# tensorlayer/HyperPose

Hardware: AMD Instinct MI355X
Metric: end-to-end FPS (preproc+DNN+PAF parse) @ 368x432 (higher is better)
Workload: dtype f32; 1 GPU; configs[1]: Lightweight-OpenPose (MobilenetDilated) + PAF parser, batch 8 @ 368x432 per GPU; frames from pinned host memory (one H2D per batch), parser on the network's own maps, humans to the host; key=configs[1]/f32, global_batch=8, parallelism=frame-sharded x1, no steady-state collective, pipes_per_gpu=4, parser_input=the network's own heat-maps

## Files before the change

hyperpose_amd/csrc/conv32_head.hip:

```cpp
#include "conv_fp32.hpp"

#include "conv_device.hpp"

#include <cstdlib>

namespace hp {

namespace {

typedef float f32x4 __attribute__((ext_vector_type(4)));

constexpr int HK1 = 128;
constexpr int HXP = (HK1 + 4) * 4;
constexpr int HX_BYTES = 32 * HXP;

__device__ __forceinline__ long tvh_off(const tview32& t, int b, int y, int x)
{
    return ((long)b * t.img + (long)y * t.wp + x) * t.cs + t.coff;
}

}

template <int TM2>
__device__ __forceinline__ void conv32_head_body(const conv32_params& q, const head32_hidden& h, unsigned char* const xs, float* const red_, const int blk)
{
    float (*const red)[TM2][4][64][4] = reinterpret_cast<float (*)[TM2][4][64][4]>(red_);

    const int tid = threadIdx.x, lane = tid & 63, wave = tid >> 6;
    const int n0 = blk * 32;
    const int OHW = q.OH * q.OW;

    {
        const int px = tid >> 3, q0 = tid & 7;
        const int n = min(n0 + px, q.npix - 1);
        const int b = n / OHW, rem = n - b * OHW;
        const int oy = rem / q.OW, ox = rem - oy * q.OW;
        const float* const src = q.in.p + tvh_off(q.in, b, oy, ox);
        f32x4 v[4];
#pragma unroll
        for (int i = 0; i < 4; ++i)
            v[i] = *reinterpret_cast<const f32x4*>(src + (q0 + 8 * i) * 4);
#pragma unroll
        for (int i = 0; i < 4; ++i)
            *reinterpret_cast<f32x4*>(xs + px * HXP + (q0 + 8 * i) * 16) = v[i];
    }
    lds_barrier();
    const int n = lane & 31, fk = lane >> 5;
    f32x4 xb[HK1 / 8];
#pragma unroll
    for (int k = 0; k < HK1 / 8; ++k)
        xb[k] = *reinterpret_cast<const f32x4*>(xs + n * HXP + (k * 8 + fk * 4) * 4);

    floatx16 acc2[TM2];
#pragma unroll
    for (int m = 0; m < TM2; ++m)
#pragma unroll
        for (int r = 0; r < 16; ++r)
            acc2[m][r] = 0.f;

    const int MT1 = h.HID / 32, nt = MT1 / 4;
    const float* const w1 = h.w1_frag + lane * 4;
    const float* const w2 = h.w2_frag + lane * 4;
    constexpr int KS = HK1 / 8, RING = 4, AHEAD = 3;
    const int nsteps = nt * KS;
    f32x4 fa[RING];
    auto aload = [&](int slot, int st) {
        const int sc = min(st, nsteps - 1), ht = wave + 4 * (sc / KS), k = sc % KS;
        fa[slot] = *reinterpret_cast<const f32x4*>(w1 + (long)(k * MT1 + ht) * 256);
    };
#pragma unroll
    for (int a = 0; a < AHEAD; ++a)
        aload(a, a);
#pragma unroll 1
    for (int it = 0; it < nt; ++it) {
        const int ht = wave + 4 * it;
        floatx16 acc1;
#pragma unroll
        for (int r = 0; r < 16; ++r)
            acc1[r] = 0.f;
        f32x4 a2[TM2][4];
#pragma unroll
        for (int m = 0; m < TM2; ++m)
#pragma unroll
            for (int qd = 0; qd < 4; ++qd)
                a2[m][qd] = *reinterpret_cast<const f32x4*>(w2 + (long)(((ht * TM2 + m) * 4 + qd) * 256));
        f32x4 bs[4];
#pragma unroll
        for (int qd = 0; qd < 4; ++qd)
            bs[qd] = *reinterpret_cast<const f32x4*>(h.bias1 + ht * 32 + 8 * qd + 4 * fk);
#pragma unroll
        for (int k = 0; k < KS; ++k) {
            aload((k + AHEAD) % RING, it * KS + k + AHEAD);
            const f32x4 a = fa[k % RING];
#pragma unroll
            for (int e = 0; e < 4; ++e)
                acc1 = __builtin_amdgcn_mfma_f32_32x32x2f32(a[e], xb[k][e], acc1, 0, 0, 0);
        }
#pragma unroll
        for (int r = 0; r < 16; ++r) {
            const float x = acc1[r] + bs[r >> 2][r & 3];
            acc1[r] = x > 0.f ? fminf(x, h.hi1) : x * h.slope1;
        }
#pragma unroll
        for (int m = 0; m < TM2; ++m)
#pragma unroll
            for (int r = 0; r < 16; ++r)
                acc2[m] = __builtin_amdgcn_mfma_f32_32x32x2f32(a2[m][r >> 2][r & 3], acc1[r], acc2[m], 0, 0, 0);
    }

#pragma unroll
    for (int m = 0; m < TM2; ++m)
#pragma unroll
        for (int qd = 0; qd < 4; ++qd)
            *reinterpret_cast<f32x4*>(&red[wave][m][qd][lane][0]) = f32x4{ acc2[m][4 * qd], acc2[m][4 * qd + 1], acc2[m][4 * qd + 2], acc2[m][4 * qd + 3] };
    lds_barrier();
    if (wave >= TM2)
        return;
    const int np = n0 + n;
    const bool pix_ok = np < q.npix;
    const int nc = min(np, q.npix - 1);
    const int b = nc / OHW, rem = nc - b * OHW;
    const int oy = rem / q.OW, ox = rem - oy * q.OW;
    const long ooff = q.out.p ? tvh_off(q.out, b, oy, ox) : 0;
    const bool out_vec = q.out.p && ((q.out.coff | q.out.cs) & 3) == 0;
#pragma unroll
    for (int qd = 0; qd < 4; ++qd) {
        f32x4 sum = *reinterpret_cast<const f32x4*>(&red[0][wave][qd][lane][0]);
#pragma unroll
        for (int w = 1; w < 4; ++w)
            sum += *reinterpret_cast<const f32x4*>(&red[w][wave][qd][lane][0]);
        const int m = wave * 32 + 8 * qd + 4 * fk;
        if (pix_ok && m < q.Cout) {
            const bool full = m + 3 < q.Cout;
            const f32x4 b2 = *reinterpret_cast<const f32x4*>(q.bias + m);
            f32x4 sl = { q.act_slope, q.act_slope, q.act_slope, q.act_slope };
            if (q.alpha)
                sl = *reinterpret_cast<const f32x4*>(q.alpha + m);
            float v[4];
#pragma unroll
            for (int e = 0; e < 4; ++e) {
                const float x = sum[e] + b2[e];
                v[e] = x > 0.f ? fminf(x, q.act_hi) : x * sl[e];
            }
            if (q.out.p) {
                if (full && out_vec)
                    *reinterpret_cast<f32x4*>(q.out.p + ooff + m) = f32x4{ v[0], v[1], v[2], v[3] };
                else {
#pragma unroll
                    for (int e = 0; e < 4; ++e)
                        if (m + e < q.Cout)
                            q.out.p[ooff + m + e] = v[e];
                }
            }
            if (q.out_f32) {
#pragma unroll
                for (int e = 0; e < 4; ++e)
                    if (m + e < q.Cout)
                        q.out_f32[((long)b * q.Cout + m + e) * OHW + rem] = v[e];
            }
        }
    }
}

template <int TM2>
__global__ __launch_bounds__(256, 2) void conv32_head_kernel(const conv32_params q, const head32_hidden h)
{
    __shared__ __attribute__((aligned(16))) unsigned char xs[HX_BYTES];
    __shared__ __attribute__((aligned(16))) float red[4 * TM2 * 4 * 64 * 4];
    conv32_head_body<TM2>(q, h, xs, red, blockIdx.x);
}

template <int TMA, int TMB>
__global__ __launch_bounds__(256, 2) void conv32_head_pair_kernel(const conv32_params qa, const head32_hidden ha, const conv32_params qb, const head32_hidden hb)
{
    __shared__ __attribute__((aligned(16))) unsigned char xs[HX_BYTES];
    __shared__ __attribute__((aligned(16))) float red[4 * (TMA > TMB ? TMA : TMB) * 4 * 64 * 4];
    const int blk = (blockIdx.x >> 4) * 8 + (blockIdx.x & 7);
    if (blk * 32 >= qa.npix)
        return;
    if ((blockIdx.x >> 3) & 1)
        conv32_head_body<TMB>(qb, hb, xs, red, blk);
    else
        conv32_head_body<TMA>(qa, ha, xs, red, blk);
}

bool conv32_head_ok(int k1, int hid, int c2) { return k1 == HK1 && hid >= 128 && hid % 128 == 0 && c2 >= 1 && c2 <= 64; }

int conv32_head_tile(int hid, int c2) { return 37000000 + hid * 100 + c2; }

void conv32_head_pack(const float* w2, int tm2, int hid, float* out)
{
    for (int ht = 0; ht < hid / 32; ++ht)
        for (int m2 = 0; m2 < tm2; ++m2)
            for (int qd = 0; qd < 4; ++qd)
                for (int lane = 0; lane < 64; ++lane)
                    for (int e = 0; e < 4; ++e)
                        out[((((size_t)ht * tm2 + m2) * 4 + qd) * 64 + lane) * 4 + e] =
                            w2[(size_t)(m2 * 32 + (lane & 31)) * hid + ht * 32 + e + 8 * qd + 4 * (lane >> 5)];
}

static bool head_args_ok(const conv32_params& q, const head32_hidden& h)
{
    return conv32_head_ok(HK1, h.HID, q.Cout) && h.w1_frag && h.w2_frag && h.bias1 && q.npix > 0 && (q.out.p || q.out_f32);
}

static bool same_input(const conv32_params& a, const conv32_params& b)
{
    return a.in.p == b.in.p && a.in.cs == b.in.cs && a.in.coff == b.in.coff && a.in.wp == b.in.wp && a.in.img == b.in.img && a.OH == b.OH && a.OW == b.OW
        && a.npix == b.npix;
}

bool conv32_head_pair_ok(const conv32_params& a, const conv32_params& b, const engine_switches& sw) { return sw.head_pair32 && same_input(a, b); }

hipError_t launch_conv32_head_pair(const conv32_params& qa, const head32_hidden& ha, const conv32_params& qb, const head32_hidden& hb, hipStream_t s)
{
    if (!head_args_ok(qa, ha) || !head_args_ok(qb, hb) || !same_input(qa, qb))
        return hipErrorInvalidValue;
    const dim3 grid(((qa.npix + 31) / 32 + 7) / 8 * 8 * 2);
    const bool a1 = qa.Cout <= 32, b1 = qb.Cout <= 32;
    if (a1 && b1)
        HP_LAUNCH((conv32_head_pair_kernel<1, 1>), grid, dim3(256), 0, s, qa, ha, qb, hb);
    else if (a1)
        HP_LAUNCH((conv32_head_pair_kernel<1, 2>), grid, dim3(256), 0, s, qa, ha, qb, hb);
    else if (b1)
        HP_LAUNCH((conv32_head_pair_kernel<2, 1>), grid, dim3(256), 0, s, qa, ha, qb, hb);
    else
        HP_LAUNCH((conv32_head_pair_kernel<2, 2>), grid, dim3(256), 0, s, qa, ha, qb, hb);
    return hipGetLastError();
}

hipError_t launch_conv32_head(const conv32_params& q, const head32_hidden& h, hipStream_t s)
{
    if (!conv32_head_ok(HK1, h.HID, q.Cout) || !h.w1_frag || !h.w2_frag || !h.bias1 || q.npix <= 0 || (!q.out.p && !q.out_f32))
        return hipErrorInvalidValue;
    const dim3 grid((q.npix + 31) / 32);
    if (q.Cout <= 32)
        HP_LAUNCH((conv32_head_kernel<1>), grid, dim3(256), 0, s, q, h);
    else
        HP_LAUNCH((conv32_head_kernel<2>), grid, dim3(256), 0, s, q, h);
    return hipGetLastError();
}

}
```

hyperpose_amd/csrc/conv_fp32.hip:

```cpp
#include "conv_fp32.hpp"

#include "conv32_epilogue.hpp"
#include "conv_device.hpp"

#include <algorithm>
#include <cstdlib>
#include <type_traits>

namespace hp {

namespace {

typedef float f32x4 __attribute__((ext_vector_type(4)));
typedef __attribute__((address_space(1))) float gfloat;
typedef __attribute__((address_space(1))) f32x4 gf32x4;

__device__ __forceinline__ float act32(float v, int act, float param, float alpha)
{
    switch (act) {
    case ACT_RELU:
        return fmaxf(v, 0.f);
    case ACT_RELU6:
        return fminf(fmaxf(v, 0.f), 6.f);
    case ACT_LEAKY:
        return v > 0.f ? v : v * param;
    case ACT_PRELU:
        return v > 0.f ? v : v * alpha;
    case ACT_SIGMOID:
        return 1.f / (1.f + expf(-v));
    case ACT_SOFTPLUS:
        return v > 20.f ? v : log1pf(expf(v));
    default:
        return v;
    }
}

__device__ __forceinline__ long tv32_off(const tview32& t, int b, int y, int x)
{
    return ((long)b * t.img + (long)y * t.wp + x) * t.cs + t.coff;
}

}

template <int BM, int BN, int WM, int WN, bool ROWS>
__global__ __launch_bounds__(256) void conv32_kernel(const conv32_params p)
{
    constexpr int BK = 16, LDR = 20;
    constexpr int TM = BM / WM / 32, TN = BN / WN / 32, NA = BM / 64, NB = BN / 64;
    static_assert(WM * WN == 4 && TM >= 1 && TN >= 1 && NA >= 1 && NB >= 1, "tile");
    constexpr int AB_BYTES = 2 * (BM + BN) * LDR * 4, SLABS = 4 * rows_geom<TM>::SLAB_BYTES;
    __shared__ __attribute__((aligned(16))) unsigned char lds_raw[AB_BYTES > SLABS ? AB_BYTES : SLABS];
    float (*const sA)[BM * LDR] = reinterpret_cast<float (*)[BM * LDR]>(lds_raw);
    float (*const sB)[BN * LDR] = reinterpret_cast<float (*)[BN * LDR]>(lds_raw + 2 * BM * LDR * 4);

    const int tid = threadIdx.x, lane = tid & 63, wave = tid >> 6;
    const int wm = wave / WN, wn = wave % WN;
    const int G = p.Cout_pad / BM, nx = (p.npix + BN - 1) / BN;
    const int bj = blockIdx.x >> 3, ptile = (bj / G) * 8 + (blockIdx.x & 7);
    if (ptile >= nx)
        return;
    const int n0 = ptile * BN, m0 = (bj % G) * BM;
    const int lrow = tid >> 2, lchunk = (tid & 3) * 4;
    const int OHW = p.OH * p.OW, kc = p.Cin / BK, steps = p.KH * p.KW * kc;

    int dbg_i = 0;
#define HP_STAMP()                                       \
    if (p.dbg && blockIdx.x == 9 && tid == 0)            \
        p.dbg[dbg_i++] = __builtin_amdgcn_s_memtime();
    HP_STAMP();
    long bbase[NB];
#pragma unroll
    for (int j = 0; j < NB; ++j) {
        const int n = min(n0 + lrow + 64 * j, p.npix - 1);
        const int b = n / OHW, rem = n - b * OHW;
        const int oy = rem / p.OW, ox = rem - oy * p.OW;
        bbase[j] = tv32_off(p.in, b, oy * p.stride - p.pad_t, ox * p.stride - p.pad_l) + lchunk;
    }
    const float* const wrow = p.w + (long)(m0 + lrow) * p.Cin + lchunk;

    f32x4 ra[NA], rb[NB];
    auto gload = [&](int s) {
        const int tap = s / kc, k0 = (s - tap * kc) * BK;
        const int ky = tap / p.KW, kx = tap - ky * p.KW;
        const long toff = ((long)(ky * p.dil) * p.in.wp + kx * p.dil) * p.in.cs + k0;
        const float* const wt = wrow + (long)tap * p.Cout_pad * p.Cin + k0;
#pragma unroll
        for (int j = 0; j < NA; ++j)
            ra[j] = *reinterpret_cast<const f32x4*>(wt + (long)(64 * j) * p.Cin);
#pragma unroll
        for (int j = 0; j < NB; ++j)
            rb[j] = *reinterpret_cast<const f32x4*>(p.in.p + bbase[j] + toff);
    };
    auto to_lds = [&](int buf) {
#pragma unroll
        for (int j = 0; j < NA; ++j)
            *reinterpret_cast<f32x4*>(&sA[buf][(lrow + 64 * j) * LDR + lchunk]) = ra[j];
#pragma unroll
        for (int j = 0; j < NB; ++j)
            *reinterpret_cast<f32x4*>(&sB[buf][(lrow + 64 * j) * LDR + lchunk]) = rb[j];
    };

    floatx16 acc[TM][TN];
#pragma unroll
    for (int i = 0; i < TM; ++i)
#pragma unroll
        for (int j = 0; j < TN; ++j)
#pragma unroll
            for (int r = 0; r < 16; ++r)
                acc[i][j][r] = 0.f;

    const int frow = lane & 31, fh = (lane >> 5) * 4;
    if (p.dbg && tid == 0 && blockIdx.x < 4096) {
        p.dbg[128 + 3 * blockIdx.x] = __builtin_amdgcn_s_memrealtime();
        p.dbg[128 + 3 * blockIdx.x + 2] = ((unsigned long long)__builtin_amdgcn_s_getreg((31 << 11) | 20) << 32) | (unsigned)__builtin_amdgcn_s_getreg((31 << 11) | 4);
    }
    gload(0);
    to_lds(0);
    lds_barrier();
    HP_STAMP();
#pragma unroll 1
    for (int s = 0; s < steps; ++s) {
        gload(min(s + 1, steps - 1));
        const float* const a_s = &sA[s & 1][(wm * TM * 32 + frow) * LDR + fh];
        const float* const b_s = &sB[s & 1][(wn * TN * 32 + frow) * LDR + fh];
#pragma unroll
        for (int kk = 0; kk < BK / 8; ++kk) {
            f32x4 fa[TM], fb[TN];
#pragma unroll
            for (int i = 0; i < TM; ++i)
                fa[i] = *reinterpret_cast<const f32x4*>(a_s + i * 32 * LDR + kk * 8);
#pragma unroll
            for (int j = 0; j < TN; ++j)
                fb[j] = *reinterpret_cast<const f32x4*>(b_s + j * 32 * LDR + kk * 8);
#pragma unroll
            for (int e = 0; e < 4; ++e)
#pragma unroll
                for (int i = 0; i < TM; ++i)
#pragma unroll
                    for (int j = 0; j < TN; ++j)
                        acc[i][j] = __builtin_amdgcn_mfma_f32_32x32x2f32(fa[i][e], fb[j][e], acc[i][j], 0, 0, 0);
        }
        to_lds((s + 1) & 1);
        lds_barrier();
        if ((s & 7) == 7)
            HP_STAMP();
    }

    if constexpr (ROWS) {
        lds_barrier();
        float* const slab = reinterpret_cast<float*>(lds_raw) + wave * (rows_geom<TM>::SLAB_BYTES / 4);
        int pn = min(n0 + wn * TN * 32 + lane / rows_geom<TM>::LPR, p.npix - 1), pb = pn / OHW;
        int poy = (pn - pb * OHW) / p.OW, pox = pn - pb * OHW - poy * p.OW;
#pragma unroll
        for (int j = 0; j < TN; ++j) {
            floatx16 fin[TM];
#pragma unroll
            for (int i = 0; i < TM; ++i)
                fin[i] = acc[i][j];
            const int nb = n0 + (wn * TN + j) * 32;
            conv32_store_rows<TM>(p, fin, slab, lane, m0 + wm * TM * 32, [&](int r, bool& ok, long& ooff, long& roff) {
                const int n = nb + r, nc = min(n, p.npix - 1);
                ok = n < p.npix;
                pox += nc - pn, pn = nc;
                while (pox >= p.OW) {
                    pox -= p.OW;
                    if (++poy == p.OH)
                        poy = 0, ++pb;
                }
// ... 422 lines not shown
#pragma unroll
                        for (int e = 0; e < 4; ++e)
                            if (m + e < p.Cout)
                                rv[e] = p.res.p[roff + e];
                    }
                }
#pragma unroll
                for (int e = 0; e < 4; ++e) {
                    float x = a[e] + bsr[h][e];
                    if (res_pre)
                        x += rv[e];
                    x = x > 0.f ? fminf(x, p.act_hi) : x * slr[h][e];
                    if (res_post)
                        x += rv[e];
                    v[e] = x;
                }
                if (full && out_vec)
                    *reinterpret_cast<f32x4*>(p.out.p + ooff) = f32x4{ v[0], v[1], v[2], v[3] };
                else {
#pragma unroll
                    for (int e = 0; e < 4; ++e)
                        if (m + e < p.Cout)
                            p.out.p[ooff + e] = v[e];
                }
            }
            __builtin_amdgcn_wave_barrier();
        }
    }
}

template <int KT, int BN>
static hipError_t launch_wk(const conv32_params& p, dim3 grid, hipStream_t s)
{
    constexpr int lds = KT / 16 * ((64 * 16 + 16) + (BN * 16 + 16)) * 4 + 4 * 16 * 36 * 4 + 3 * BN * 8;
    static bool granted = false;
    if (lds > 64 * 1024 && !granted) {
        const hipError_t e = hipFuncSetAttribute((const void*)conv32_wk_kernel<KT, BN>, hipFuncAttributeMaxDynamicSharedMemorySize, lds);
        if (e != hipSuccess)
            return e;
        granted = true;
    }
    HP_LAUNCH((conv32_wk_kernel<KT, BN>), grid, dim3(256), lds, s, p);
    return hipGetLastError();
}

static int conv32_wk_bn(const conv32_params& p, const engine_switches& sw)
{
    const int wk = sw.c32_wk;
    if (wk == 0 || p.KH != 1 || p.KW != 1 || p.dil != 1 || p.out_f32 || !p.out.p || (p.Cin != 32 && p.Cin != 64 && p.Cin != 128))
        return 0;
    if (p.Cin == 128 && wk != 1)
        return 0;
    const int bn = 64;
    const long np = p.pick_npix > 0 ? p.pick_npix : p.npix, blocks = (np + bn - 1) / bn * (p.Cout_pad / 64);
    return wk == 1 || blocks >= 768 ? bn : 0;
}

static void conv32_pick(const conv32_params& p, const engine_switches& sw, int& BM, int& BN)
{
    BM = p.Cout_pad % 128 == 0 ? 128 : 64, BN = 128;
    const long blocks = (long)(((p.pick_npix > 0 ? p.pick_npix : p.npix) + 127) / 128) * (p.Cout_pad / BM);
    if (blocks < 448)
        BM = 64, BN = 64;
    else if (blocks < 1024 && BM == 128)
        BM = 64;
    const int bn160 = sw.c32_bn160;
    if (bn160 == 1 || bn160 == 176) {
        BM = 64, BN = bn160 == 1 ? 160 : 176;
        return;
    }
    if (BM == 64 && BN == 128 && bn160 != 0) {
        const long np = p.pick_npix > 0 ? p.pick_npix : p.npix;
        const long g = p.Cout_pad / 64, b128 = (long)((np + 127) / 128) * g, b160 = (long)((np + 159) / 160) * g;
        if (b128 > 1024 && b160 <= 1024)
            BN = 160;
    }
    if (bn160 != 0 && p.KH == 1 && p.KW == 1 && p.stride == 1 && p.Cin <= 128 && p.Cout_pad >= 256 && !p.out_f32 && (BN == 128))
        BM = 64, BN = 160;
}

static bool conv32_rows(const conv32_params& p, int BN)
{
    if (BN == 160 || BN == 176)
        return false;
    return !p.out_f32 && (p.lane_epilogue < 0 || (p.lane_epilogue == 0 && BN == 64));
}

int conv32_tile(const conv32_params& p, const engine_switches& sw)
{
    if (const int bn = conv32_wk_bn(p, sw))
        return 39000000 + p.Cin * 1000 + bn;
    int BM, BN;
    conv32_pick(p, sw, BM, BN);
    return 32000000 + (conv32_rows(p, BN) ? 400000 : 0) + BM * 1000 + BN;
}

bool set_act32(conv32_params& p)
{
    const float inf = __builtin_huge_valf();
    switch (p.act) {
    case ACT_NONE:
        p.act_slope = 1.f, p.act_hi = inf;
        return true;
    case ACT_RELU:
        p.act_slope = 0.f, p.act_hi = inf;
        return true;
    case ACT_RELU6:
        p.act_slope = 0.f, p.act_hi = 6.f;
        return true;
    case ACT_LEAKY:
        p.act_slope = p.act_param, p.act_hi = inf;
        return true;
    case ACT_PRELU:
        p.act_slope = 0.f, p.act_hi = inf;
        return p.alpha != nullptr;
    default:
        return false;
    }
}

hipError_t launch_conv32(const conv32_params& p, const engine_switches& sw, hipStream_t s)
{
    if (p.Cin % 16 || p.Cout_pad % 64 || p.npix <= 0)
        return hipErrorInvalidValue;
    if (const int bn = conv32_wk_bn(p, sw)) {
        const dim3 g(((p.npix + bn - 1) / bn + 7) / 8 * 8 * (p.Cout_pad / 64));
        return p.Cin == 32 ? launch_wk<32, 64>(p, g, s) : p.Cin == 64 ? launch_wk<64, 64>(p, g, s) : launch_wk<128, 64>(p, g, s);
    }
    int BM, BN;
    conv32_pick(p, sw, BM, BN);
    const dim3 grid(((p.npix + BN - 1) / BN + 7) / 8 * 8 * (p.Cout_pad / BM));
    const bool rows = conv32_rows(p, BN);
#define HP_C32_CASE(BM_, BN_, WM_, WN_)                                                    \
    if (rows)                                                                              \
        HP_LAUNCH((conv32_kernel<BM_, BN_, WM_, WN_, true>), grid, dim3(256), 0, s, p);    \
    else                                                                                   \
        HP_LAUNCH((conv32_kernel<BM_, BN_, WM_, WN_, false>), grid, dim3(256), 0, s, p);
    if (BN == 176) {
        HP_LAUNCH((conv32_t16_kernel<176, 1>), grid, dim3(256), 0, s, p);
    } else if (BN == 160) {
        HP_LAUNCH((conv32_t16_kernel<160>), grid, dim3(256), 0, s, p);
    } else if (BM == 128) {
        HP_C32_CASE(128, 128, 2, 2)
    } else if (BN == 128) {
        HP_C32_CASE(64, 128, 1, 4)
    } else {
        HP_C32_CASE(64, 64, 2, 2)
    }
#undef HP_C32_CASE
    return hipGetLastError();
}

__device__ unsigned g_first_conv_verify[4];
__global__ __launch_bounds__(256) void first_conv32_kernel(const first_conv32_params p, int tiles_x, int tiles_y, int TH, int GP, int verify)
{
    extern __shared__ __attribute__((aligned(16))) float s_w32[];
    constexpr int TW = 8, PX = 4;
    const int G = (p.Cout + 7) / 8, CP = G * 8, taps = p.KH * p.KW;
    const int IH = (TH - 1) * p.stride + p.KH, IW = (TW - 1) * p.stride + p.KW;
    float* const s_x = s_w32 + taps * 3 * CP;
    int t = blockIdx.x;
    const int tx = t % tiles_x;
    t /= tiles_x;
    const int ty = t % tiles_y, b = t / tiles_y;
    const int oy0 = ty * TH, ox0 = tx * TW;
    const int iy0 = oy0 * p.stride - p.pad_t, ix0 = ox0 * p.stride - p.pad_l;
    for (int i = threadIdx.x; i < taps * 3 * CP; i += 256) {
        const int co = i % CP, tc = i / CP;
        s_w32[i] = co < p.Cout ? p.w[(size_t)co * taps * 3 + tc] : 0.f;
    }
    for (int i = threadIdx.x; i < IH * IW; i += 256) {
        const int py = i / IW, px = i - py * IW;
        const int iy = iy0 + py, ix = ix0 + px;
        float v[3] = { 0.f, 0.f, 0.f };
        if (iy >= 0 && iy < p.H && ix >= 0 && ix < p.W) {
            if (p.in_u8) {
                const uint8_t* q = p.in_u8 + (((size_t)b * p.H + iy) * p.W + ix) * 3;
#pragma unroll
                for (int c = 0; c < 3; ++c)
                    v[c] = ((float)((double)q[p.flip_rb ? 2 - c : c] * p.factor) - p.mean[c]) * p.inv_std[c];
            } else {
#pragma unroll
                for (int c = 0; c < 3; ++c)
                    v[c] = (p.in_f32[(((size_t)b * 3 + c) * p.H + iy) * p.W + ix] - p.mean[c]) * p.inv_std[c];
            }
        }
        s_x[i * 3] = v[0], s_x[i * 3 + 1] = v[1], s_x[i * 3 + 2] = v[2];
    }
    __syncthreads();
    const int g0 = threadIdx.x % GP, slot = threadIdx.x / GP;
    auto verify_lds = [&]() {
        if (!verify)
            return;
        unsigned bad_x = 0, bad_w = 0;
        for (int i = threadIdx.x; i < IH * IW; i += 256) {
            const int py = i / IW, px = i - py * IW;
            const int iy = iy0 + py, ix = ix0 + px;
            float v[3] = { 0.f, 0.f, 0.f };
            if (iy >= 0 && iy < p.H && ix >= 0 && ix < p.W && p.in_u8) {
                const uint8_t* q = p.in_u8 + (((size_t)b * p.H + iy) * p.W + ix) * 3;
                for (int c = 0; c < 3; ++c)
                    v[c] = ((float)((double)q[p.flip_rb ? 2 - c : c] * p.factor) - p.mean[c]) * p.inv_std[c];
            }
            for (int c = 0; c < 3; ++c)
                bad_x += __float_as_uint(s_x[i * 3 + c]) != __float_as_uint(v[c]);
        }
        for (int i = threadIdx.x; i < taps * 3 * CP; i += 256) {
            const int co = i % CP, tc = i / CP;
            const float wv = co < p.Cout ? p.w[(size_t)co * taps * 3 + tc] : 0.f;
            bad_w += __float_as_uint(s_w32[i]) != __float_as_uint(wv);
        }
        if (bad_x)
            atomicAdd(&g_first_conv_verify[0], bad_x);
        if (bad_w)
            atomicAdd(&g_first_conv_verify[1], bad_w);
        if (threadIdx.x == 0)
            atomicAdd(&g_first_conv_verify[2], 1u);
    };
    if (slot >= TH * (TW / PX)) {
        verify_lds();
        return;
    }
    const int ly = slot / (TW / PX), lx0 = (slot % (TW / PX)) * PX;
    const int oy = oy0 + ly;
    if (oy >= p.OH) {
        verify_lds();
        return;
    }
    const bool vec_ok = ((p.out.coff | p.out.cs) & 3) == 0;
    for (int g = g0; g < G; g += GP) {
        float acc[PX][8];
#pragma unroll
        for (int r = 0; r < 8; ++r) {
            const float bv = (g * 8 + r < p.Cout) ? p.bias[g * 8 + r] : 0.f;
#pragma unroll
            for (int j = 0; j < PX; ++j)
                acc[j][r] = bv;
        }
        for (int ky = 0; ky < p.KH; ++ky)
            for (int kx = 0; kx < p.KW; ++kx) {
                const float* xp = s_x + ((ly * p.stride + ky) * IW + lx0 * p.stride + kx) * 3;
                const float* wt = s_w32 + (size_t)((ky * p.KW + kx) * 3) * CP + g * 8;
#pragma unroll
                for (int c = 0; c < 3; ++c) {
                    const f32x4 w0 = *reinterpret_cast<const f32x4*>(wt + c * CP);
                    const f32x4 w1 = *reinterpret_cast<const f32x4*>(wt + c * CP + 4);
#pragma unroll
                    for (int j = 0; j < PX; ++j) {
                        const float xv = xp[j * p.stride * 3 + c];
#pragma unroll
                        for (int e = 0; e < 4; ++e)
                            acc[j][e] = fmaf(xv, w0[e], acc[j][e]), acc[j][4 + e] = fmaf(xv, w1[e], acc[j][4 + e]);
                    }
                }
            }
        if (verify) {
            float acc2[PX][8];
#pragma unroll
            for (int r = 0; r < 8; ++r) {
                const float bv = (g * 8 + r < p.Cout) ? p.bias[g * 8 + r] : 0.f;
#pragma unroll
                for (int j = 0; j < PX; ++j)
                    acc2[j][r] = bv;
            }
            for (int ky = 0; ky < p.KH; ++ky)
                for (int kx = 0; kx < p.KW; ++kx) {
                    const float* xp = s_x + ((ly * p.stride + ky) * IW + lx0 * p.stride + kx) * 3;
                    const float* wt = s_w32 + (size_t)((ky * p.KW + kx) * 3) * CP + g * 8;
#pragma unroll
                    for (int c = 0; c < 3; ++c) {
                        const f32x4 w0 = *reinterpret_cast<const f32x4*>(wt + c * CP);
                        const f32x4 w1 = *reinterpret_cast<const f32x4*>(wt + c * CP + 4);
#pragma unroll
                        for (int j = 0; j < PX; ++j) {
                            const float xv = xp[j * p.stride * 3 + c];
#pragma unroll
                            for (int e = 0; e < 4; ++e)
                                acc2[j][e] = fmaf(xv, w0[e], acc2[j][e]), acc2[j][4 + e] = fmaf(xv, w1[e], acc2[j][4 + e]);
                        }
                    }
                }
            unsigned bad = 0;
#pragma unroll
            for (int j = 0; j < PX; ++j)
#pragma unroll
                for (int r = 0; r < 8; ++r)
                    bad += __float_as_uint(acc[j][r]) != __float_as_uint(acc2[j][r]);
            if (bad)
                atomicAdd(&g_first_conv_verify[3], bad);
        }
#pragma unroll
        for (int j = 0; j < PX; ++j) {
            const int ox = ox0 + lx0 + j;
            if (ox >= p.OW)
                break;
            float* op = p.out.p + tv32_off(p.out, b, oy, ox) + g * 8;
            if (g * 8 + 7 < p.Cout && vec_ok) {
                f32x4 o0, o1;
#pragma unroll
                for (int e = 0; e < 4; ++e)
                    o0[e] = act32(acc[j][e], p.act, p.act_param, 0.f), o1[e] = act32(acc[j][4 + e], p.act, p.act_param, 0.f);
                *reinterpret_cast<f32x4*>(op) = o0, *reinterpret_cast<f32x4*>(op + 4) = o1;
            } else {
#pragma unroll
                for (int r = 0; r < 8; ++r)
                    if (g * 8 + r < p.Cout)
                        op[r] = act32(acc[j][r], p.act, p.act_param, 0.f);
            }
        }
    }
    verify_lds();
}

void first_conv32_verify_counts(unsigned out[4], bool reset)
{
    (void)hipMemcpyFromSymbol(out, HIP_SYMBOL(g_first_conv_verify), 16);
    if (reset) {
        const unsigned z[4] = { 0, 0, 0, 0 };
        (void)hipMemcpyToSymbol(HIP_SYMBOL(g_first_conv_verify), z, 16);
    }
}

hipError_t launch_first_conv32(const first_conv32_params& p, const engine_switches& sw, hipStream_t s)
{
    const int G = (p.Cout + 7) / 8, GP = std::min(G, 32);
    const int TH = 256 / GP / 2;
    const int IH = (TH - 1) * p.stride + p.KH, IW = 7 * p.stride + p.KW;
    const size_t lds = ((size_t)p.KH * p.KW * 3 * G * 8 + (size_t)IH * IW * 3) * sizeof(float);
    if (lds > 64 * 1024)
        return hipErrorInvalidValue;
    const int tiles_x = (p.OW + 7) / 8, tiles_y = (p.OH + TH - 1) / TH;
    HP_LAUNCH(first_conv32_kernel, dim3(tiles_x * tiles_y * p.B), dim3(256), lds, s, p, tiles_x, tiles_y, TH, GP, sw.first_conv_verify ? 1 : 0);
    return hipGetLastError();
}

template <int S, int D, int PX>
__global__ __launch_bounds__(256) void dwconv32_kernel(const dw32_params p, int run)
{
    static_assert(PX == 1 || (PX == 2 && S == 1), "column pairs share taps at stride 1 only");
    constexpr int NR = 2 * D + 1;
    constexpr int NC = 2 + PX;
    const int CG = p.C / 4, segs = (p.OH + run - 1) / run;
    const int ncol = PX == 1 ? p.OW : (p.OW + 2 * D - 1) / (2 * D) * D;
    const long total = (long)p.B * segs * ncol * CG;
    for (long i = (long)blockIdx.x * 256 + threadIdx.x; i < total; i += (long)gridDim.x * 256) {
        const int cg = (int)(i % CG);
        long n = i / CG;
        const int q = (int)(n % ncol);
        n /= ncol;
        const int ox = PX == 1 ? q : (q / D) * 2 * D + q % D;
        if (ox >= p.OW)
            continue;
        const int seg = (int)(n % segs), b = (int)(n / segs);
        const int oy0 = seg * run, oy1 = min(oy0 + run, p.OH);
        f32x4 w[9];
#pragma unroll
        for (int t = 0; t < 9; ++t)
            w[t] = *reinterpret_cast<const f32x4*>(p.w + t * p.C + cg * 4);
        const f32x4 bias = *reinterpret_cast<const f32x4*>(p.bias + cg * 4);
        const int cx0 = ox * S - p.pad_l, cmax = p.W - 1 + (2 * D - p.pad_l);
        long coff[NC];
#pragma unroll
        for (int c = 0; c < NC; ++c)
            coff[c] = (long)(min(cx0 + c * D, cmax) - cx0) * p.in.cs;
        const float* const col0 = p.in.p + tv32_off(p.in, b, oy0 * S - p.pad_t, cx0) + cg * 4;
        const long rstride = (long)p.in.wp * p.in.cs;
        f32x4 x[NR][NC];
        auto load_row = [&](int r, long row) {
#pragma unroll
            for (int c = 0; c < NC; ++c)
                x[r][c] = *reinterpret_cast<const f32x4*>(col0 + row * rstride + coff[c]);
        };
#pragma unroll
        for (int r = 0; r < NR; ++r)
            load_row(r, r);
        float* op = p.out.p + tv32_off(p.out, b, oy0, ox) + cg * 4;
        const long ostride = (long)p.out.wp * p.out.cs, o2 = (long)D * p.out.cs;
        const bool second = PX == 2 && ox + D < p.OW;
        for (int oy = oy0; oy < oy1; ++oy) {
#pragma unroll
            for (int px = 0; px < PX; ++px) {
                f32x4 acc = bias;
#pragma unroll
                for (int ky = 0; ky < 3; ++ky)
#pragma unroll
                    for (int kx = 0; kx < 3; ++kx)
#pragma unroll
                        for (int e = 0; e < 4; ++e)
                            acc[e] = fmaf(x[ky * D][kx + px][e], w[ky * 3 + kx][e], acc[e]);
                f32x4 o;
#pragma unroll
                for (int e = 0; e < 4; ++e)
                    o[e] = act32(acc[e], p.act, p.act_param, 0.f);
                if (px == 0 || second)
                    *reinterpret_cast<f32x4*>(op + px * o2) = o;
            }
            op += ostride;
#pragma unroll
            for (int r = 0; r + S < NR; ++r)
#pragma unroll
                for (int c = 0; c < NC; ++c)
                    x[r][c] = x[r + S][c];
            if (oy + 1 < oy1) {
#pragma unroll
                for (int r = NR - S; r < NR; ++r)
                    load_row(r, (long)(oy + 1 - oy0) * S + r);
            }
        }
    }
}

__global__ __launch_bounds__(256) void dwconv32_any_kernel(const dw32_params p)
{
    const int CG = p.C / 4;
    const long total = (long)p.B * p.OH * p.OW * CG;
    for (long i = (long)blockIdx.x * 256 + threadIdx.x; i < total; i += (long)gridDim.x * 256) {
        const int cg = (int)(i % CG);
        const long n = i / CG;
        const int ox = (int)(n % p.OW);
        const long t = n / p.OW;
        const int oy = (int)(t % p.OH), b = (int)(t / p.OH);
        f32x4 acc = *reinterpret_cast<const f32x4*>(p.bias + cg * 4);
        const float* const x0 = p.in.p + tv32_off(p.in, b, oy * p.stride - p.pad_t, ox * p.stride - p.pad_l) + cg * 4;
#pragma unroll
        for (int ky = 0; ky < 3; ++ky)
#pragma unroll
            for (int kx = 0; kx < 3; ++kx) {
                const f32x4 x = *reinterpret_cast<const f32x4*>(x0 + ((long)(ky * p.dil) * p.in.wp + kx * p.dil) * p.in.cs);
                const f32x4 w = *reinterpret_cast<const f32x4*>(p.w + (ky * 3 + kx) * p.C + cg * 4);
#pragma unroll
                for (int e = 0; e < 4; ++e)
                    acc[e] = fmaf(x[e], w[e], acc[e]);
            }
        f32x4 o;
#pragma unroll
        for (int e = 0; e < 4; ++e)
            o[e] = act32(acc[e], p.act, p.act_param, 0.f);
        *reinterpret_cast<f32x4*>(p.out.p + tv32_off(p.out, b, oy, ox) + cg * 4) = o;
    }
}

hipError_t launch_dwconv32(const dw32_params& p, const engine_switches& sw, hipStream_t s)
{
    if (p.C % 4)
        return hipErrorInvalidValue;
    const int run = p.OH >= 32 ? 8 : 4;
    const int px_env = sw.dw32_px;
    const bool pairs = px_env != 1;
    const long pair_threads = (long)p.B * ((p.OH + run - 1) / run) * ((p.OW + 2 * p.dil - 1) / (2 * p.dil) * p.dil) * (p.C / 4);
    const bool two = pairs && p.stride == 1 && (p.dil == 1 || p.dil == 2) && (pair_threads >= 120000 || px_env == 2);
    const int ncol = two ? (p.OW + 2 * p.dil - 1) / (2 * p.dil) * p.dil : p.OW;
    const long total = (long)p.B * ((p.OH + run - 1) / run) * ncol * (p.C / 4);
    const int blocks = (int)std::min<long>((total + 255) / 256, 256 * 32);
    if (p.stride == 1 && p.dil == 1) {
        if (two)
            HP_LAUNCH((dwconv32_kernel<1, 1, 2>), dim3(blocks), dim3(256), 0, s, p, run);
        else
            HP_LAUNCH((dwconv32_kernel<1, 1, 1>), dim3(blocks), dim3(256), 0, s, p, run);
    } else if (p.stride == 2 && p.dil == 1)
        HP_LAUNCH((dwconv32_kernel<2, 1, 1>), dim3(blocks), dim3(256), 0, s, p, run);
    else if (p.stride == 1 && p.dil == 2) {
        if (two)
            HP_LAUNCH((dwconv32_kernel<1, 2, 2>), dim3(blocks), dim3(256), 0, s, p, run);
        else
            HP_LAUNCH((dwconv32_kernel<1, 2, 1>), dim3(blocks), dim3(256), 0, s, p, run);
    }
    else {
        const long px = (long)p.B * p.OH * p.OW * (p.C / 4);
        HP_LAUNCH(dwconv32_any_kernel, dim3((int)std::min<long>((px + 255) / 256, 256 * 32)), dim3(256), 0, s, p);
    }
    return hipGetLastError();
}

__global__ __launch_bounds__(256) void maxpool32_kernel(const pool32_params p)
{
    const int CG = p.C / 4;
    const long total = (long)p.B * p.OH * p.OW * CG;
    for (long i = (long)blockIdx.x * 256 + threadIdx.x; i < total; i += (long)gridDim.x * 256) {
        const int cg = (int)(i % CG);
        const long n = i / CG;
        const int ox = (int)(n % p.OW);
        const long t = n / p.OW;
        const int oy = (int)(t % p.OH), b = (int)(t / p.OH);
        f32x4 m = { -__builtin_huge_valf(), -__builtin_huge_valf(), -__builtin_huge_valf(), -__builtin_huge_valf() };
        for (int ky = 0; ky < p.k; ++ky) {
// ... 108 lines not shown
```

Measured before the change: 5450 frames/s.

## Pipeline head-conv LDS/weight loads and specialise first conv for fixed kernel shapes

In the fused head kernel, the activation fragments are now streamed from LDS one k-step ahead instead of being held in registers. The weight prefetch ring is deepened and explicit sched_group_barrier interleaving is added. The epilogue now runs on all waves, with bias and slope loads hoisted and output offsets precomputed. The first conv is templated on 3x3/7x7 stride-2 with a padded LDS pitch, word-wide u8 staging and register-cached input rows. These changes add register pressure and rigid scheduling constraints that could hurt occupancy.

Result: no change. 5497 frames/s (median of 6 runs) (+0.9%).

```diff
diff --git a/hyperpose_amd/csrc/conv32_head.hip b/hyperpose_amd/csrc/conv32_head.hip
--- a/hyperpose_amd/csrc/conv32_head.hip
+++ b/hyperpose_amd/csrc/conv32_head.hip
@@ -9,6 +9,8 @@
 namespace {
 
 typedef float f32x4 __attribute__((ext_vector_type(4)));
+typedef __attribute__((address_space(1))) float gfloath;
+typedef __attribute__((address_space(1))) f32x4 gf32x4h;
 
 constexpr int HK1 = 128;
 constexpr int HXP = (HK1 + 4) * 4;
@@ -46,10 +48,7 @@
     }
     lds_barrier();
     const int n = lane & 31, fk = lane >> 5;
-    f32x4 xb[HK1 / 8];
-#pragma unroll
-    for (int k = 0; k < HK1 / 8; ++k)
-        xb[k] = *reinterpret_cast<const f32x4*>(xs + n * HXP + (k * 8 + fk * 4) * 4);
+    unsigned xrow = (unsigned)(n * HXP + fk * 16);
 
     floatx16 acc2[TM2];
 #pragma unroll
@@ -61,19 +60,32 @@
     const int MT1 = h.HID / 32, nt = MT1 / 4;
     const float* const w1 = h.w1_frag + lane * 4;
     const float* const w2 = h.w2_frag + lane * 4;
-    constexpr int KS = HK1 / 8, RING = 4, AHEAD = 3;
+    constexpr int KS = HK1 / 8, RING = 8, AHEAD = 6;
+    static_assert(KS % RING == 0, "the ring position is a compile-time function of k");
     const int nsteps = nt * KS;
     f32x4 fa[RING];
     auto aload = [&](int slot, int st) {
         const int sc = min(st, nsteps - 1), ht = wave + 4 * (sc / KS), k = sc % KS;
-        fa[slot] = *reinterpret_cast<const f32x4*>(w1 + (long)(k * MT1 + ht) * 256);
+        fa[slot] = *(const gf32x4h*)(w1 + (long)(k * MT1 + ht) * 256);
     };
 #pragma unroll
     for (int a = 0; a < AHEAD; ++a)
         aload(a, a);
+
+    const int np = n0 + n;
+    const bool pix_ok = np < q.npix;
+    const int nc = min(np, q.npix - 1);
+    const int ob = nc / OHW, orem = nc - ob * OHW;
+    const int ooy = orem / q.OW, oox = orem - ooy * q.OW;
+    const long ooff = q.out.p ? tvh_off(q.out, ob, ooy, oox) : 0;
+    const long foff = (long)ob * q.Cout * OHW + orem;
+    const bool out_vec = q.out.p && ((q.out.coff | q.out.cs) & 3) == 0;
+    const int dq = 8 * wave + 4 * fk;
+    f32x4 xn = *reinterpret_cast<const f32x4*>(xs + xrow);
 #pragma unroll 1
     for (int it = 0; it < nt; ++it) {
         const int ht = wave + 4 * it;
+        asm volatile("" : "+v"(xrow));
         floatx16 acc1;
 #pragma unroll
         for (int r = 0; r < 16; ++r)
@@ -83,18 +95,27 @@
         for (int m = 0; m < TM2; ++m)
 #pragma unroll
             for (int qd = 0; qd < 4; ++qd)
-                a2[m][qd] = *reinterpret_cast<const f32x4*>(w2 + (long)(((ht * TM2 + m) * 4 + qd) * 256));
+                a2[m][qd] = *(const gf32x4h*)(w2 + (long)(((ht * TM2 + m) * 4 + qd) * 256));
         f32x4 bs[4];
 #pragma unroll
         for (int qd = 0; qd < 4; ++qd)
-            bs[qd] = *reinterpret_cast<const f32x4*>(h.bias1 + ht * 32 + 8 * qd + 4 * fk);
+            bs[qd] = *(const gf32x4h*)(h.bias1 + ht * 32 + 8 * qd + 4 * fk);
+        __builtin_amdgcn_sched_barrier(0);
 #pragma unroll
         for (int k = 0; k < KS; ++k) {
+            const f32x4 xb = xn;
+            xn = *reinterpret_cast<const f32x4*>(xs + xrow + ((k + 1) % KS) * 32);
             aload((k + AHEAD) % RING, it * KS + k + AHEAD);
             const f32x4 a = fa[k % RING];
 #pragma unroll
             for (int e = 0; e < 4; ++e)
-                acc1 = __builtin_amdgcn_mfma_f32_32x32x2f32(a[e], xb[k][e], acc1, 0, 0, 0);
+                acc1 = __builtin_amdgcn_mfma_f32_32x32x2f32(a[e], xb[e], acc1, 0, 0, 0);
+            __builtin_amdgcn_sched_group_barrier(0x008, 1, 0);
+            __builtin_amdgcn_sched_group_barrier(0x100, 1, 0);
+            __builtin_amdgcn_sched_group_barrier(0x008, 1, 0);
+            __builtin_amdgcn_sched_group_barrier(0x020, 1, 0);
+            __builtin_amdgcn_sched_group_barrier(0x008, 2, 0);
+            __builtin_amdgcn_sched_barrier(0);
         }
 #pragma unroll
         for (int r = 0; r < 16; ++r) {
@@ -108,57 +129,66 @@
                 acc2[m] = __builtin_amdgcn_mfma_f32_32x32x2f32(a2[m][r >> 2][r & 3], acc1[r], acc2[m], 0, 0, 0);
     }
 
+    f32x4 b2[TM2], sl2[TM2];
+#pragma unroll
+    for (int j = 0; j < TM2; ++j) {
+        const int m = 32 * j + dq, mc = m < q.Cout ? m : 0;
+        b2[j] = *(const gf32x4h*)(q.bias + mc);
+        sl2[j] = f32x4{ q.act_slope, q.act_slope, q.act_slope, q.act_slope };
+        if (q.alpha)
+            sl2[j] = *(const gf32x4h*)(q.alpha + mc);
+    }
 #pragma unroll
     for (int m = 0; m < TM2; ++m)
 #pragma unroll
         for (int qd = 0; qd < 4; ++qd)
             *reinterpret_cast<f32x4*>(&red[wave][m][qd][lane][0]) = f32x4{ acc2[m][4 * qd], acc2[m][4 * qd + 1], acc2[m][4 * qd + 2], acc2[m][4 * qd + 3] };
     lds_barrier();
-    if (wave >= TM2)
-        return;
-    const int np = n0 + n;
-    const bool pix_ok = np < q.npix;
-    const int nc = min(np, q.npix - 1);
-    const int b = nc / OHW, rem = nc - b * OHW;
-    const int oy = rem / q.OW, ox = rem - oy * q.OW;
-    const long ooff = q.out.p ? tvh_off(q.out, b, oy, ox) : 0;
-    const bool out_vec = q.out.p && ((q.out.coff | q.out.cs) & 3) == 0;
-#pragma unroll
-    for (int qd = 0; qd < 4; ++qd) {
-        f32x4 sum = *reinterpret_cast<const f32x4*>(&red[0][wave][qd][lane][0]);
+    f32x4 v[TM2];
+#pragma unroll
+    for (int j = 0; j < TM2; ++j) {
+        f32x4 sum = *reinterpret_cast<const f32x4*>(&red[0][j][wave][lane][0]);
 #pragma unroll
         for (int w = 1; w < 4; ++w)
-            sum += *reinterpret_cast<const f32x4*>(&red[w][wave][qd][lane][0]);
-        const int m = wave * 32 + 8 * qd + 4 * fk;
-        if (pix_ok && m < q.Cout) {
-            const bool full = m + 3 < q.Cout;
-            const f32x4 b2 = *reinterpret_cast<const f32x4*>(q.bias + m);
-            f32x4 sl = { q.act_slope, q.act_slope, q.act_slope, q.act_slope };
-            if (q.alpha)
-                sl = *reinterpret_cast<const f32x4*>(q.alpha + m);
-            float v[4];
-#pragma unroll
-            for (int e = 0; e < 4; ++e) {
-                const float x = sum[e] + b2[e];
-                v[e] = x > 0.f ? fminf(x, q.act_hi) : x * sl[e];
-            }
-            if (q.out.p) {
-                if (full && out_vec)
-                    *reinterpret_cast<f32x4*>(q.out.p + ooff + m) = f32x4{ v[0], v[1], v[2], v[3] };
-                else {
-#pragma unroll
-                    for (int e = 0; e < 4; ++e)
+            sum += *reinterpret_cast<const f32x4*>(&red[w][j][wave][lane][0]);
+#pragma unroll
+        for (int e = 0; e < 4; ++e) {
+            const float x = sum[e] + b2[j][e];
+            v[j][e] = x > 0.f ? fminf(x, q.act_hi) : x * sl2[j][e];
+        }
+    }
+    if (q.out.p) {
+        gfloath* const op = (gfloath*)q.out.p + ooff;
+        if (out_vec) {
+#pragma unroll
+            for (int j = 0; j < TM2; ++j) {
+                const int m = 32 * j + dq;
+                if (pix_ok && m + 3 < q.Cout)
+                    *reinterpret_cast<gf32x4h*>(op + m) = v[j];
+                else if (pix_ok) {
+#pragma unroll
+                    for (int e = 0; e < 3; ++e)
                         if (m + e < q.Cout)
-                            q.out.p[ooff + m + e] = v[e];
+                            op[m + e] = v[j][e];
                 }
             }
-            if (q.out_f32) {
+        } else {
+#pragma unroll
+            for (int j = 0; j < TM2; ++j)
 #pragma unroll
                 for (int e = 0; e < 4; ++e)
-                    if (m + e < q.Cout)
-                        q.out_f32[((long)b * q.Cout + m + e) * OHW + rem] = v[e];
-            }
-        }
+                    if (pix_ok && 32 * j + dq + e < q.Cout)
+                        op[32 * j + dq + e] = v[j][e];
+        }
+    }
+    if (q.out_f32) {
+        gfloath* const fp = (gfloath*)q.out_f32 + foff;
+#pragma unroll
+        for (int j = 0; j < TM2; ++j)
+#pragma unroll
+            for (int e = 0; e < 4; ++e)
+                if (pix_ok && 32 * j + dq + e < q.Cout)
+                    fp[(long)(32 * j + dq + e) * OHW] = v[j][e];
     }
 }
 
diff --git a/hyperpose_amd/csrc/conv_fp32.hip b/hyperpose_amd/csrc/conv_fp32.hip
--- a/hyperpose_amd/csrc/conv_fp32.hip
+++ b/hyperpose_amd/csrc/conv_fp32.hip
@@ -14,6 +14,8 @@
 typedef float f32x4 __attribute__((ext_vector_type(4)));
 typedef __attribute__((address_space(1))) float gfloat;
 typedef __attribute__((address_space(1))) f32x4 gf32x4;
+typedef __attribute__((address_space(1))) unsigned char guchar;
+typedef __attribute__((address_space(1), aligned(1))) unsigned gu32_any;
 
 __device__ __forceinline__ float act32(float v, int act, float param, float alpha)
 {
@@ -742,45 +744,110 @@
 }
 
 __device__ unsigned g_first_conv_verify[4];
-__global__ __launch_bounds__(256) void first_conv32_kernel(const first_conv32_params p, int tiles_x, int tiles_y, int TH, int GP, int verify)
+template <int KH_, int KW_, int S_, bool VERIFY>
+__global__ __launch_bounds__(256) void first_conv32_kernel(const first_conv32_params p, int tiles_x, int tiles_y, int TH, int GP)
 {
     extern __shared__ __attribute__((aligned(16))) float s_w32[];
+    constexpr bool FIX = KH_ != 0;
     constexpr int TW = 8, PX = 4;
-    const int G = (p.Cout + 7) / 8, CP = G * 8, taps = p.KH * p.KW;
-    const int IH = (TH - 1) * p.stride + p.KH, IW = (TW - 1) * p.stride + p.KW;
+    const int KH = FIX ? KH_ : p.KH, KW = FIX ? KW_ : p.KW, stride = FIX ? S_ : p.stride;
+    const int G = (p.Cout + 7) / 8, CP = G * 8, taps = KH * KW;
+    const int IH = (TH - 1) * stride + KH, IW = (TW - 1) * stride + KW;
+    const int PITCH = FIX ? (IW * 3 + 3) / 4 * 4 : IW * 3;
     float* const s_x = s_w32 + taps * 3 * CP;
     int t = blockIdx.x;
     const int tx = t % tiles_x;
     t /= tiles_x;
     const int ty = t % tiles_y, b = t / tiles_y;
     const int oy0 = ty * TH, ox0 = tx * TW;
-    const int iy0 = oy0 * p.stride - p.pad_t, ix0 = ox0 * p.stride - p.pad_l;
-    for (int i = threadIdx.x; i < taps * 3 * CP; i += 256) {
-        const int co = i % CP, tc = i / CP;
-        s_w32[i] = co < p.Cout ? p.w[(size_t)co * taps * 3 + tc] : 0.f;
-    }
-    for (int i = threadIdx.x; i < IH * IW; i += 256) {
-        const int py = i / IW, px = i - py * IW;
-        const int iy = iy0 + py, ix = ix0 + px;
-        float v[3] = { 0.f, 0.f, 0.f };
-        if (iy >= 0 && iy < p.H && ix >= 0 && ix < p.W) {
-            if (p.in_u8) {
-                const uint8_t* q = p.in_u8 + (((size_t)b * p.H + iy) * p.W + ix) * 3;
-#pragma unroll
-                for (int c = 0; c < 3; ++c)
-                    v[c] = ((float)((double)q[p.flip_rb ? 2 - c : c] * p.factor) - p.mean[c]) * p.inv_std[c];
-            } else {
-#pragma unroll
-                for (int c = 0; c < 3; ++c)
-                    v[c] = (p.in_f32[(((size_t)b * 3 + c) * p.H + iy) * p.W + ix] - p.mean[c]) * p.inv_std[c];
-            }
-        }
-        s_x[i * 3] = v[0], s_x[i * 3 + 1] = v[1], s_x[i * 3 + 2] = v[2];
+    const int iy0 = oy0 * stride - p.pad_t, ix0 = ox0 * stride - p.pad_l;
+    const float mean0 = p.mean[0], mean1 = p.mean[1], mean2 = p.mean[2], istd0 = p.inv_std[0], istd1 = p.inv_std[1], istd2 = p.inv_std[2];
+    const auto stage_pixels = [&]() {
+        for (int i = threadIdx.x; i < IH * IW; i += 256) {
+            const int py = i / IW, px = i - py * IW;
+            const int iy = iy0 + py, ix = ix0 + px;
+            float v[3] = { 0.f, 0.f, 0.f };
+            if (iy >= 0 && iy < p.H && ix >= 0 && ix < p.W) {
+                if (p.in_u8) {
+                    const uint8_t* q = p.in_u8 + (((size_t)b * p.H + iy) * p.W + ix) * 3;
+#pragma unroll
+                    for (int c = 0; c < 3; ++c)
+                        v[c] = ((float)((double)q[p.flip_rb ? 2 - c : c] * p.factor) - p.mean[c]) * p.inv_std[c];
+                } else {
+#pragma unroll
+                    for (int c = 0; c < 3; ++c)
+                        v[c] = (p.in_f32[(((size_t)b * 3 + c) * p.H + iy) * p.W + ix] - p.mean[c]) * p.inv_std[c];
+                }
+            }
+            float* const d = s_x + py * PITCH + px * 3;
+            d[0] = v[0], d[1] = v[1], d[2] = v[2];
+        }
+    };
+    if constexpr (FIX) {
+        constexpr int TC = KH_ * KW_ * 3, UN = 4;
+        constexpr int IWc = (TW - 1) * S_ + KW_, RB = IWc * 3, NW = (RB + 3) / 4;
+        const int nwt = TC * CP, nwords = p.in_u8 ? IH * NW : 0;
+        const int vlo = max(0, -ix0) * 3, vhi = min(IWc, p.W - ix0) * 3;
+        const long total = (long)p.B * p.H * p.W * 3;
+        const gfloat* const gw = (const gfloat*)p.w;
+        const guchar* const gin = (const guchar*)p.in_u8;
+        for (int base = threadIdx.x; base < max(nwt, nwords); base += 256 * UN) {
+            float wv[UN];
+            unsigned pw[UN] = { 0, 0, 0, 0 };
+            int sh[UN] = { 0, 0, 0, 0 };
+#pragma unroll
+            for (int u = 0; u < UN; ++u)
+                wv[u] = gw[min(base + u * 256, nwt - 1)];
+            if (nwords) {
+#pragma unroll
+                for (int u = 0; u < UN; ++u) {
+                    const int i = min(base + u * 256, nwords - 1), py = i / NW, e0 = (i - py * NW) * 4, iy = iy0 + py;
+                    const bool row_ok = iy >= 0 && iy < p.H;
+                    const long want = row_ok ? (((long)b * p.H + iy) * p.W + ix0) * 3 + e0 : 0;
+                    const long at = want < 0 ? 0 : want > total - 4 ? total - 4 : want;
+                    pw[u] = *(const gu32_any*)(gin + at);
+                    sh[u] = (int)(want - at) * 8;
+                }
+            }
+            __builtin_amdgcn_sched_barrier(0);
+#pragma unroll
+            for (int u = 0; u < UN; ++u) {
+                const int i = base + u * 256, co = i / TC, tc = i - co * TC;
+                if (i < nwt)
+                    s_w32[tc * CP + co] = wv[u];
+            }
+#pragma unroll
+            for (int u = 0; u < UN; ++u) {
+                const int i = base + u * 256, py = i / NW, e0 = (i - py * NW) * 4, iy = iy0 + py;
+                const bool row_ok = iy >= 0 && iy < p.H;
+                if (i >= nwords)
+                    continue;
+                const unsigned wd = sh[u] >= 0 ? pw[u] >> (sh[u] & 31) : pw[u] << (-sh[u] & 31);
+#pragma unroll
+                for (int k = 0; k < 4; ++k) {
+                    const int e = e0 + k;
+                    if (e >= RB)
+                        break;
+                    const int px = e / 3, sc = e - px * 3, c = p.flip_rb ? 2 - sc : sc;
+                    const float mean = c == 0 ? mean0 : c == 1 ? mean1 : mean2, istd = c == 0 ? istd0 : c == 1 ? istd1 : istd2;
+                    const float v = ((float)((double)((wd >> (8 * k)) & 255u) * p.factor) - mean) * istd;
+                    s_x[py * PITCH + px * 3 + c] = (row_ok && e >= vlo && e < vhi) ? v : 0.f;
+                }
+            }
+        }
+        if (!p.in_u8)
+            stage_pixels();
+    } else {
+        for (int i = threadIdx.x; i < taps * 3 * CP; i += 256) {
+            const int co = i % CP, tc = i / CP;
+            s_w32[i] = co < p.Cout ? p.w[(size_t)co * taps * 3 + tc] : 0.f;
+        }
+        stage_pixels();
     }
     __syncthreads();
     const int g0 = threadIdx.x % GP, slot = threadIdx.x / GP;
     auto verify_lds = [&]() {
-        if (!verify)
+        if constexpr (!VERIFY)
             return;
         unsigned bad_x = 0, bad_w = 0;
         for (int i = threadIdx.x; i < IH * IW; i += 256) {
@@ -793,7 +860,7 @@
                     v[c] = ((float)((double)q[p.flip_rb ? 2 - c : c] * p.factor) - p.mean[c]) * p.inv_std[c];
             }
             for (int c = 0; c < 3; ++c)
-                bad_x += __float_as_uint(s_x[i * 3 + c]) != __float_as_uint(v[c]);
+                bad_x += __float_as_uint(s_x[py * PITCH + px * 3 + c]) != __float_as_uint(v[c]);
         }
         for (int i = threadIdx.x; i < taps * 3 * CP; i += 256) {
             const int co = i % CP, tc = i / CP;
@@ -819,57 +886,67 @@
     }
     const bool vec_ok = ((p.out.coff | p.out.cs) & 3) == 0;
     for (int g = g0; g < G; g += GP) {
-        float acc[PX][8];
-#pragma unroll
-        for (int r = 0; r < 8; ++r) {
-            const float bv = (g * 8 + r < p.Cout) ? p.bias[g * 8 + r] : 0.f;
-#pragma unroll
-            for (int j = 0; j < PX; ++j)
-                acc[j][r] = bv;
-        }
-        for (int ky = 0; ky < p.KH; ++ky)
-            for (int kx = 0; kx < p.KW; ++kx) {
-                const float* xp = s_x + ((ly * p.stride + ky) * IW + lx0 * p.stride + kx) * 3;
-                const float* wt = s_w32 + (size_t)((ky * p.KW + kx) * 3) * CP + g * 8;
-#pragma unroll
-                for (int c = 0; c < 3; ++c) {
-                    const f32x4 w0 = *reinterpret_cast<const f32x4*>(wt + c * CP);
-                    const f32x4 w1 = *reinterpret_cast<const f32x4*>(wt + c * CP + 4);
-#pragma unroll
-                    for (int j = 0; j < PX; ++j) {
-                        const float xv = xp[j * p.stride * 3 + c];
-#pragma unroll
-                        for (int e = 0; e < 4; ++e)
-                            acc[j][e] = fmaf(xv, w0[e], acc[j][e]), acc[j][4 + e] = fmaf(xv, w1[e], acc[j][4 + e]);
-                    }
-                }
-            }
-        if (verify) {
-            float acc2[PX][8];
+        auto run_taps = [&](float (&acc)[PX][8]) {
 #pragma unroll
             for (int r = 0; r < 8; ++r) {
-                const float bv = (g * 8 + r < p.Cout) ? p.bias[g * 8 + r] : 0.f;
+                const float bv = (FIX || g * 8 + r < p.Cout) ? p.bias[g * 8 + r] : 0.f;
 #pragma unroll
                 for (int j = 0; j < PX; ++j)
-                    acc2[j][r] = bv;
-            }
-            for (int ky = 0; ky < p.KH; ++ky)
-                for (int kx = 0; kx < p.KW; ++kx) {
-                    const float* xp = s_x + ((ly * p.stride + ky) * IW + lx0 * p.stride + kx) * 3;
-                    const float* wt = s_w32 + (size_t)((ky * p.KW + kx) * 3) * CP + g * 8;
-#pragma unroll
-                    for (int c = 0; c < 3; ++c) {
-                        const f32x4 w0 = *reinterpret_cast<const f32x4*>(wt + c * CP);
-                        const f32x4 w1 = *reinterpret_cast<const f32x4*>(wt + c * CP + 4);
+                    acc[j][r] = bv;
+            }
+            if constexpr (FIX) {
+                constexpr int ROWF = ((PX - 1) * S_ + KW_) * 3, NR = (ROWF + 3) / 4;
+                static_assert((PX * S_ * 3) % 4 == 0, "the right half's window starts on a quad");
+                static_assert(PX * S_ * 3 + NR * 4 <= (((TW - 1) * S_ + KW_) * 3 + 3) / 4 * 4, "whole quads stay inside the padded row");
+                const float* const xrow = s_x + ly * S_ * PITCH + lx0 * S_ * 3;
+                const float* wt = s_w32 + g * 8;
+                f32x4 wn0 = *reinterpret_cast<const f32x4*>(wt), wn1 = *reinterpret_cast<const f32x4*>(wt + 4);
+#pragma unroll 1
+                for (int ky = 0; ky < KH_; ++ky) {
+                    f32x4 xr[NR];
+#pragma unroll
+                    for (int i = 0; i < NR; ++i)
+                        xr[i] = *reinterpret_cast<const f32x4*>(xrow + ky * PITCH + 4 * i);
+#pragma unroll
+                    for (int kc = 0; kc < KW_ * 3; ++kc) {
+                        const f32x4 w0 = wn0, w1 = wn1;
+                        wt += CP;
+                        wn0 = *reinterpret_cast<const f32x4*>(wt), wn1 = *reinterpret_cast<const f32x4*>(wt + 4);
+                        __builtin_amdgcn_sched_barrier(0);
 #pragma unroll
                         for (int j = 0; j < PX; ++j) {
-                            const float xv = xp[j * p.stride * 3 + c];
+                            const float xv = xr[(j * S_ * 3 + kc) >> 2][(j * S_ * 3 + kc) & 3];
 #pragma unroll
                             for (int e = 0; e < 4; ++e)
-                                acc2[j][e] = fmaf(xv, w0[e], acc2[j][e]), acc2[j][4 + e] = fmaf(xv, w1[e], acc2[j][4 + e]);
+                                acc[j][e] = fmaf(xv, w0[e], acc[j][e]), acc[j][4 + e] = fmaf(xv, w1[e], acc[j][4 + e]);
                         }
                     }
                 }
+            } else {
+                for (int ky = 0; ky < KH; ++ky)
+                    for (int kx = 0; kx < KW; ++kx) {
+                        const float* xp = s_x + (ly * stride + ky) * PITCH + (lx0 * stride + kx) * 3;
+                        const float* wt = s_w32 + (size_t)((ky * KW + kx) * 3) * CP + g * 8;
+#pragma unroll
+                        for (int c = 0; c < 3; ++c) {
+                            const f32x4 w0 = *reinterpret_cast<const f32x4*>(wt + c * CP);
+                            const f32x4 w1 = *reinterpret_cast<const f32x4*>(wt + c * CP + 4);
+#pragma unroll
+                            for (int j = 0; j < PX; ++j) {
+                                const float xv = xp[j * stride * 3 + c];
+#pragma unroll
+                                for (int e = 0; e < 4; ++e)
+                                    acc[j][e] = fmaf(xv, w0[e], acc[j][e]), acc[j][4 + e] = fmaf(xv, w1[e], acc[j][4 + e]);
+                            }
+                        }
+                    }
+            }
+        };
+        float acc[PX][8];
+        run_taps(acc);
+        if constexpr (VERIFY) {
+            float acc2[PX][8];
+            run_taps(acc2);
             unsigned bad = 0;
 #pragma unroll
             for (int j = 0; j < PX; ++j)
@@ -916,11 +993,26 @@
     const int G = (p.Cout + 7) / 8, GP = std::min(G, 32);
     const int TH = 256 / GP / 2;
     const int IH = (TH - 1) * p.stride + p.KH, IW = 7 * p.stride + p.KW;
-    const size_t lds = ((size_t)p.KH * p.KW * 3 * G * 8 + (size_t)IH * IW * 3) * sizeof(float);
+    const auto lds_bytes = [&](int pitch) { return ((size_t)p.KH * p.KW * 3 * G * 8 + (size_t)IH * pitch) * sizeof(float); };
+    const bool fix = p.Cout % 8 == 0 && p.H * p.W >= 2 && p.stride == 2 && p.KH == p.KW && (p.KH == 3 || p.KH == 7) && lds_bytes((IW * 3 + 3) / 4 * 4) <= 64 * 1024;
+    const size_t lds = lds_bytes(fix ? (IW * 3 + 3) / 4 * 4 : IW * 3);
     if (lds > 64 * 1024)
         return hipErrorInvalidValue;
     const int tiles_x = (p.OW + 7) / 8, tiles_y = (p.OH + TH - 1) / TH;
-    HP_LAUNCH(first_conv32_kernel, dim3(tiles_x * tiles_y * p.B), dim3(256), lds, s, p, tiles_x, tiles_y, TH, GP, sw.first_conv_verify ? 1 : 0);
+    const dim3 grid(tiles_x * tiles_y * p.B);
+#define HP_FIRST32_CASE(KH_, KW_, S_)                                                                                   \
+    if (sw.first_conv_verify)                                                                                           \
+        HP_LAUNCH((first_conv32_kernel<KH_, KW_, S_, true>), grid, dim3(256), lds, s, p, tiles_x, tiles_y, TH, GP);     \
+    else                                                                                                                \
+        HP_LAUNCH((first_conv32_kernel<KH_, KW_, S_, false>), grid, dim3(256), lds, s, p, tiles_x, tiles_y, TH, GP);
+    if (fix && p.KH == 3) {
+        HP_FIRST32_CASE(3, 3, 2)
+    } else if (fix) {
+        HP_FIRST32_CASE(7, 7, 2)
+    } else {
+        HP_FIRST32_CASE(0, 0, 0)
+    }
+#undef HP_FIRST32_CASE
     return hipGetLastError();
 }
 
```
